# 0xEigenLabs/eigen-zkvm

Hardware: AMD Instinct MI355X
Metric: Goldilocks NTT GElems/s + BN254 G1 MSM Mpts/s; starky prove ms at 2^24 rows (higher is better)
Workload: dtype u64 (Goldilocks, canonical)

## Files before the change

eigen-zkvm_amd/csrc/ntt.hip:

```cpp
#include "zk_internal.h"
#include "ntt_reg.hip.h"
#include <map>
#include <mutex>
#include <vector>

namespace zk {

namespace {

constexpr int NTT_TILE = 4096;
constexpr int TW_LO_BITS = 12;
constexpr int TW_LO = 1 << TW_LO_BITS;

struct PassParams {
    const u64* in;
    u64* out;
    const u64* w256;
    const u64* tw_lo;
    const u64* tw_hi;
    const u64* tw_mid;
    u64 pre_scale;
    u32 dshift;
    const u64* sc_lo;
    const u64* sc_hi;
    u64 sc_step;
    u64 out_scale;
    u64 inner;
    u64 valid_in;
    u64 s_np;
    u32 np;
    u32 log_s;
    u32 has_tw;
};

__device__ __forceinline__ u64 tab2(const u64* __restrict__ lo, const u64* __restrict__ hi, u64 e) {
    return gl::mul_tw_nc(hi[e >> TW_LO_BITS], lo[e & (TW_LO - 1)]);
}

template <int LOGA, int LOGB, bool KMODE, bool INV>
__global__ __launch_bounds__(NTT_TILE / 16) void ntt_pass_kernel(const PassParams P) {
    constexpr int LOGR = LOGA + LOGB, R = 1 << LOGR, RA = 1 << LOGA, RB = 1 << LOGB;
    constexpr int C = NTT_TILE / R;
    constexpr int GA = 16 / RA, GB = 16 / RB;
    constexpr int TG = R / 16;
    constexpr int PAD = KMODE ? 512 / R : 0;
    constexpr int ROW = RB * C + PAD;
    static_assert(LOGR >= 4 && LOGR <= 8 && LOGA <= 4 && LOGB <= 4, "tile shape");
    __shared__ u64 lds[RA * ROW];

    const int t = threadIdx.x;
    const u64 u0 = (u64)blockIdx.x * C;

    {
        const int c = t % C, ta = t / C;
        const u64 u = u0 + c;
        const bool live = u < P.inner;
        u64 x[GA][RA];
        const bool full = u0 + C <= P.inner && (u64)(R - 1) * P.inner + u0 + C <= P.valid_in;
        const u64* __restrict__ base = P.in + (u64)(ta * GA) * P.inner + (live ? u : 0);
        if (full) {
#pragma unroll
            for (int g = 0; g < GA; ++g)
#pragma unroll
                for (int ja = 0; ja < RA; ++ja) x[g][ja] = base[(u64)(ja * RB + g) * P.inner];
        } else {
#pragma unroll
            for (int g = 0; g < GA; ++g)
#pragma unroll
                for (int ja = 0; ja < RA; ++ja) {
                    const u64 off = (u64)(ja * RB + g) * P.inner;
                    const bool ok = live && (u64)(ta * GA) * P.inner + off + u < P.valid_in;
                    const u64 v = *(ok ? base + off : P.in);
                    x[g][ja] = ok ? v : 0;
                }
        }
#pragma unroll
        for (int g = 0; g < GA; ++g) ntt_reg<LOGA, INV>(x[g]);
        if (LOGR <= 6 && C >= 64 && LOGB > 0 && P.pre_scale == 1) {
            static_for<0, TG>([&](auto TA) {
                constexpr int ta_c = decltype(TA)::value;
                if (ta == ta_c) {
                    static_for<0, GA>([&](auto GI) {
                        constexpr int g = decltype(GI)::value, jb = ta_c * GA + g;
                        static_for<0, RA>([&](auto KA) {
                            constexpr int ka = decltype(KA)::value;
                            constexpr int e0 = (39 * (64 / (R > 64 ? 64 : R)) * jb * ka) % 192, e = INV ? (192 - e0) % 192 : e0;
                            u64 v = x[g][bitrev_c(ka, LOGA)];
                            if constexpr (e >= 96) v = gl::neg(gl::mul_pow2<e - 96>(v));
                            else v = gl::mul_pow2<e>(v);
                            lds[ka * ROW + jb * C + c] = v;
                        });
                    });
                }
            });
        } else
        {
#pragma unroll
            for (int g = 0; g < GA; ++g) {
                const int jb = ta * GA + g;
#pragma unroll
                for (int ka = 0; ka < RA; ++ka) {
                    u64 v = x[g][bitrev_c(ka, LOGA)];
                    if (LOGB > 0 && ka > 0) v = gl::mul_tw(v, P.w256[(jb * ka) << (8 - LOGR)]);
                    else if (P.pre_scale != 1) v = gl::mul_tw(v, P.pre_scale);
                    lds[ka * ROW + jb * C + c] = v;
                }
            }
        }
    }
    __syncthreads();
    {
        int c, tb;
        if (KMODE) { tb = t % TG; c = t / TG; } else { c = t % C; tb = t / C; }
        const u64 u = u0 + c;
        u64 y[GB][RB];
#pragma unroll
        for (int g = 0; g < GB; ++g) {
            const int ka = tb + g * TG;
#pragma unroll
            for (int jb = 0; jb < RB; ++jb) y[g][jb] = lds[ka * ROW + jb * C + c];
        }
        const u64 uc = u < P.inner ? u : 0;
        u64 p, rem;
        if (P.np == 1) { p = uc >> P.log_s; rem = uc & (((u64)1 << P.log_s) - 1); }
        else if ((P.inner >> 32) == 0) { const u32 p32 = (u32)uc / (u32)P.s_np; p = p32; rem = (u32)uc - p32 * (u32)P.s_np; }
        else
        { p = uc / P.s_np; rem = uc - p * P.s_np; }
        u64 tw[GB][RB];
        if (P.tw_mid) {
#pragma unroll
            for (int g = 0; g < GB; ++g) {
                const int ka = tb + g * TG;
#pragma unroll
                for (int kb = 0; kb < RB; ++kb) tw[g][kb] = P.tw_mid[((p * (u64)(RA * kb + ka)) << P.log_s) >> P.dshift];
            }
        }
#pragma unroll
        for (int g = 0; g < GB; ++g) ntt_reg<LOGB, INV>(y[g]);
        if (u >= P.inner) return;

        u64* __restrict__ outp = P.out + p * R * P.s_np + rem;
        const u64 kstride = P.s_np;
        const u64 row_q = !P.sc_lo ? 0 : P.np == 1 ? rem : (P.inner >> 32) == 0 ? (u64)((u32)rem / P.np) : rem / P.np;
        if (P.tw_mid) {
#pragma unroll
            for (int g = 0; g < GB; ++g) {
                const int ka = tb + g * TG;
#pragma unroll
                for (int kb = 0; kb < RB; ++kb) {
                    u64 v = y[g][bitrev_c(kb, LOGB)];
                    v = gl::mul_tw(v, tw[g][kb]);
                    outp[(u64)(RA * kb + ka) * kstride] = v;
                }
            }
            return;
        }
        u64 tw_step = 1;
        if (P.has_tw) tw_step = tab2(P.tw_lo, P.tw_hi, (p * RA) << P.log_s);
#pragma unroll
        for (int g = 0; g < GB; ++g) {
            const int ka = tb + g * TG;
            u64 f = P.out_scale;
            if (P.has_tw) f = tab2(P.tw_lo, P.tw_hi, (p * ka) << P.log_s);
            if (P.sc_lo) f = tab2(P.sc_lo, P.sc_hi, ((u64)ka << P.log_s) + row_q);
            const bool scaled = P.has_tw || P.sc_lo || P.out_scale != 1;
            const u64 fstep = P.sc_lo ? P.sc_step : tw_step;
#pragma unroll
            for (int kb = 0; kb < RB; ++kb) {
                u64 v = y[g][bitrev_c(kb, LOGB)];
                if (scaled) {
                    v = gl::mul_tw(v, f);
                    if (kb + 1 < RB) f = gl::mul_tw_nc(f, fstep);
                }
                outp[(u64)(RA * kb + ka) * kstride] = v;
            }
        }
    }
}

__global__ void ntt_small_kernel(const u64* in, u64* out, u32 np, u32 n_in, u32 n, u64 w, u64 g, u64 cst) {
    const u32 tid = blockIdx.x * blockDim.x + threadIdx.x;
    if (tid >= n * np) return;
    const u32 k = tid / np, c = tid % np;
    const u64 wk = gl::pow(w, k);
    u64 acc = 0, cur = 1;
    for (u32 i = 0; i < n_in; ++i) { acc = gl::add(acc, gl::mul(in[(u64)i * np + c], cur)); cur = gl::mul(cur, wk); }
    out[(u64)k * np + c] = gl::mul(acc, gl::mul(cst, gl::pow(g, k)));
}

struct Tables { DevConst w256, w256s, lo, hi, mid; u32 dshift = 0; };
struct ScaleTables { DevConst lo, hi; };

std::mutex g_mu;
auto& g_tables = *new std::map<std::pair<int, std::pair<u32, int>>, Tables>;
auto& g_scales = *new std::map<std::pair<int, std::pair<u32, u64>>, ScaleTables>;

void two_level(u64 base, u64 cst, u32 nbits, std::vector<u64>& lo, std::vector<u64>& hi) {
    lo.resize(TW_LO);
    u64 c = cst;
    for (int i = 0; i < TW_LO; ++i) { lo[i] = c; c = gl::hmul(c, base); }
    size_t nh = nbits > (u32)TW_LO_BITS ? (size_t)1 << (nbits - TW_LO_BITS) : 1;
    hi.resize(nh);
    u64 step = gl::hpow(base, TW_LO);
    c = 1;
    for (size_t i = 0; i < nh; ++i) { hi[i] = c; c = gl::hmul(c, step); }
}

const Tables& get_tables(u32 nbits, bool inverse) {
    int dev; ZK_HIP(hipGetDevice(&dev));
    std::lock_guard<std::mutex> lk(g_mu);
    auto key = std::make_pair(dev, std::make_pair(nbits, (int)inverse));
    auto it = g_tables.find(key);
    if (it != g_tables.end()) return it->second;
    u64 w = gl::hroot(nbits), w8 = gl::hroot(8);
    if (inverse) { w = gl::hinv(w); w8 = gl::hinv(w8); }
    std::vector<u64> t256(256), lo, hi;
    u64 c = 1;
    for (int i = 0; i < 256; ++i) { t256[i] = c; c = gl::hmul(c, w8); }
    two_level(w, 1, nbits, lo, hi);
    Tables T; T.w256 = DevConst(t256); T.lo = DevConst(lo); T.hi = DevConst(hi);
    if (inverse) {
        const u64 ninv = gl::hinv((1ull << nbits) % GL_P);
        std::vector<u64> t256s(256);
        for (int i = 0; i < 256; ++i) t256s[i] = gl::hmul(t256[i], ninv);
        T.w256s = DevConst(t256s);
    }
    {
        T.dshift = nbits > 16 ? nbits - 16 : 0;
        const size_t nm = (size_t)1 << (nbits - T.dshift);
        std::vector<u64> mid(nm);
        const u64 step = gl::hpow(w, 1ull << T.dshift);
        c = 1;
        for (size_t i = 0; i < nm; ++i) { mid[i] = c; c = gl::hmul(c, step); }
        T.mid = DevConst(mid);
    }
    return g_tables.emplace(key, std::move(T)).first->second;
}

const ScaleTables& get_scale(u32 nbits, u64 g, u64 cst) {
    int dev; ZK_HIP(hipGetDevice(&dev));
    std::lock_guard<std::mutex> lk(g_mu);
    auto key = std::make_pair(dev, std::make_pair(nbits, g));
    auto it = g_scales.find(key);
    if (it != g_scales.end()) return it->second;
    std::vector<u64> lo, hi;
    two_level(g, cst, nbits, lo, hi);
    ScaleTables S; S.lo = DevConst(lo); S.hi = DevConst(hi);
    return g_scales.emplace(key, std::move(S)).first->second;
}

template <int LOGA, int LOGB>
void launch_pass(const PassParams& P, bool kmode, bool inverse, hipStream_t st) {
    constexpr int C = NTT_TILE >> (LOGA + LOGB);
    const u64 blocks = (P.inner + C - 1) / C;
    ZK_REQUIRE(blocks < (1ull << 31), "ntt: grid too large");
    const dim3 g((u32)blocks), b(NTT_TILE / 16);
    const int variant = (kmode ? 2 : 0) | (inverse ? 1 : 0);
#define ZK_PASS(K, I) hipLaunchKernelGGL((ntt_pass_kernel<LOGA, LOGB, K, I>), g, b, 0, st, P)
    switch (variant) {
        case 0: ZK_PASS(false, false); break; case 1: ZK_PASS(false, true); break;
        case 2: ZK_PASS(true, false); break;  default: ZK_PASS(true, true); break;
    }
#undef ZK_PASS
    ZK_HIP(hipGetLastError());
}

void launch_pass_logr(int logr, const PassParams& P, bool kmode, bool inverse, hipStream_t st) {
    switch (logr) {
        case 4: launch_pass<2, 2>(P, kmode, inverse, st); break;
        case 5: launch_pass<3, 2>(P, kmode, inverse, st); break;
        case 6: launch_pass<3, 3>(P, kmode, inverse, st); break;
        case 7: launch_pass<4, 3>(P, kmode, inverse, st); break;
        case 8: launch_pass<4, 4>(P, kmode, inverse, st); break;
        default: throw Error("ntt: unsupported pass radix");
    }
}

std::vector<int> plan(u32 nbits) {
    std::vector<int> r;
    if (nbits < 4) return r;
    int np = (nbits + 7) / 8;
    int base = nbits / np, extra = nbits % np;
    for (int i = 0; i < np; ++i) r.push_back(base + (i < extra ? 1 : 0));
    return r;
}

struct Scale { bool on = false; u64 g = 1, cst = 1; };

void run_transform(const u64* in, u64* a, u64* b,
                   u32 n_pols, u32 nbits, u64 valid_rows, bool inverse, Scale sc, u64 out_scale, hipStream_t st) {
    const u64 n = 1ull << nbits;
    if (nbits < 4) {
        u64 w = gl::hroot(nbits);
        if (inverse) w = gl::hinv(w);
        u64 cst = sc.on ? sc.cst : out_scale;
        u64 g = sc.on ? sc.g : 1;
        u32 total = (u32)(n * n_pols);
        hipLaunchKernelGGL(ntt_small_kernel, dim3((total + 255) / 256), dim3(256), 0, st, in, a, n_pols,
                           (u32)valid_rows, (u32)n, w, g, cst);
        ZK_HIP(hipGetLastError());
        return;
    }
    const std::vector<int> radices = plan(nbits);
    const int np = (int)radices.size();
    const Tables& T = get_tables(nbits, inverse);
    const ScaleTables* S = sc.on ? &get_scale(nbits, sc.g, sc.cst) : nullptr;
    u32 log_s = 0;
    const u64* cur = in;
    for (int i = 0; i < np; ++i) {
        const int logr = radices[i];
        u64* dstbuf = ((np - 1 - i) % 2 == 0) ? a : b;
        const bool last = (i == np - 1);
        PassParams P{};
        P.in = cur; P.out = dstbuf;
        P.w256 = T.w256.u(); P.tw_lo = T.lo.u(); P.tw_hi = T.hi.u();
        P.sc_lo = (last && sc.on) ? S->lo.u() : nullptr;
        P.sc_hi = (last && sc.on) ? S->hi.u() : nullptr;
        const int loga = (logr + 1) / 2;
        P.sc_step = (last && sc.on) ? gl::hpow(sc.g, (1ull << loga) << log_s) : 1;
        P.out_scale = 1; P.pre_scale = 1;
        if (last && !sc.on && out_scale != 1) {
            ZK_REQUIRE(inverse && out_scale == gl::hinv(n % GL_P), "ntt: unsupported constant scaling");
            P.w256 = T.w256s.u(); P.pre_scale = out_scale;
        }
        P.inner = (n >> logr) * n_pols;
        P.valid_in = (i == 0) ? valid_rows * n_pols : n * n_pols;
        P.s_np = ((u64)1 << log_s) * n_pols;
        P.np = n_pols;
        P.log_s = log_s;
        P.has_tw = last ? 0 : 1;
        P.dshift = T.dshift;
        P.tw_mid = (!last && log_s >= T.dshift) ? T.mid.u() : nullptr;
        const bool kmode = P.s_np < 16;
        launch_pass_logr(logr, P, kmode, inverse, st);
        cur = dstbuf;
        log_s += logr;
    }
}

}

int ntt_num_passes(uint32_t nbits) { return nbits < 4 ? 1 : (int)plan(nbits).size(); }

const u64* ntt_w256_table(bool inverse) { return get_tables(8, inverse).w256.u(); }

void ntt_dev(const u64* d_src, u64* d_dst, u64* d_tmp, uint32_t n_pols, uint32_t nbits, bool inverse, hipStream_t st) {
    ZK_REQUIRE(nbits <= 32, "ntt: nbits > 32");
    if (n_pols == 0) return;
    ZK_REQUIRE(d_src != d_dst, "ntt: dst may not alias src");
    u64 out_scale = inverse ? gl::hinv((1ull << nbits) % GL_P) : 1;
    run_transform(d_src, d_dst, d_tmp, n_pols, nbits, 1ull << nbits, inverse, Scale{}, out_scale, st);
}

void lde_dev(const u64* d_src, u64* d_dst, u64* d_tmp, uint32_t n_pols, uint32_t nbits, uint32_t nbits_ext, hipStream_t st) {
    ZK_REQUIRE(nbits_ext <= 32 && nbits <= nbits_ext, "lde: need nbits <= nbits_ext <= 32");
    if (n_pols == 0) return;
    ZK_REQUIRE(d_src != d_dst, "lde: dst may not alias src");
    const u64 n = 1ull << nbits;
    Scale sc; sc.on = true; sc.g = 49; sc.cst = gl::hinv(n % GL_P);
    const int fwd_passes = ntt_num_passes(nbits_ext);
    u64* first_fwd_out = ((fwd_passes - 1) % 2 == 0) ? d_dst : d_tmp;
    u64* coef = (first_fwd_out == d_dst) ? d_tmp : d_dst;
    u64* other = (coef == d_dst) ? d_tmp : d_dst;
    run_transform(d_src, coef, other, n_pols, nbits, n, true, sc, 1, st);
    run_transform(coef, d_dst, d_tmp, n_pols, nbits_ext, n, false, Scale{}, 1, st);
}

}
```

Before: 81.06.

## Prefetch twiddle/scale factors before first stage and break serial factor chain

Issues the global-table loads for the output twiddle/coset factors right after the input loads, so their latency overlaps the first radix stage. Per-column step factors are precomputed cooperatively into a new shared array, replacing the serial per-kb multiply chain with independent multiplies. The scale step is now derived from a table entry times the inverse of the constant. It also adds 32-bit byte-offset addressing for tw_mid loads and for output stores when the problem is small. Costs are extra LDS and registers per block, which may lower occupancy.

```diff
diff --git a/eigen-zkvm_amd/csrc/ntt.hip b/eigen-zkvm_amd/csrc/ntt.hip
--- a/eigen-zkvm_amd/csrc/ntt.hip
+++ b/eigen-zkvm_amd/csrc/ntt.hip
@@ -2,6 +2,7 @@
 #include "ntt_reg.hip.h"
 #include <map>
 #include <mutex>
+#include <type_traits>
 #include <vector>
 
 namespace zk {
@@ -23,7 +24,7 @@
     u32 dshift;
     const u64* sc_lo;
     const u64* sc_hi;
-    u64 sc_step;
+    u64 sc_cinv;
     u64 out_scale;
     u64 inner;
     u64 valid_in;
@@ -47,9 +48,50 @@
     constexpr int ROW = RB * C + PAD;
     static_assert(LOGR >= 4 && LOGR <= 8 && LOGA <= 4 && LOGB <= 4, "tile shape");
     __shared__ u64 lds[RA * ROW];
+    __shared__ u64 sfac[RB * C];
 
     const int t = threadIdx.x;
     const u64 u0 = (u64)blockIdx.x * C;
+
+    auto split = [&](u64 u, u64& p, u64& rem) {
+        const u64 uc = u < P.inner ? u : 0;
+        if (P.np == 1) { p = uc >> P.log_s; rem = uc & (((u64)1 << P.log_s) - 1); }
+        else if ((P.inner >> 32) == 0) { const u32 p32 = (u32)uc / (u32)P.s_np; p = p32; rem = (u32)uc - p32 * (u32)P.s_np; }
+        else
+        { p = uc / P.s_np; rem = uc - p * P.s_np; }
+    };
+    auto row_of = [&](u64 rem) { return P.np == 1 ? rem : (P.inner >> 32) == 0 ? (u64)((u32)rem / P.np) : rem / P.np; };
+    const bool small = ((P.inner * R) >> 29) == 0;
+    int cB, tb;
+    if (KMODE) { tb = t % TG; cB = t / TG; } else { cB = t % C; tb = t / C; }
+
+    const bool split_f = (P.has_tw && !P.tw_mid) || P.sc_lo;
+    u64 fa_hi[GB], fa_lo[GB], fs_hi[GA], fs_lo[GA], fa[GB];
+#pragma unroll
+    for (int g = 0; g < GB; ++g) fa_hi[g] = fa_lo[g] = fa[g] = 1;
+#pragma unroll
+    for (int m = 0; m < GA; ++m) fs_hi[m] = fs_lo[m] = 1;
+    auto issue_factor_loads = [&]() {
+        const u64* __restrict__ lo = P.sc_lo ? P.sc_lo : P.tw_lo;
+        const u64* __restrict__ hi = P.sc_lo ? P.sc_hi : P.tw_hi;
+        u64 p, rem;
+        split(u0 + cB, p, rem);
+        const u32 rq = P.sc_lo ? (u32)row_of(rem) : 0;
+#pragma unroll
+        for (int g = 0; g < GB; ++g) {
+            const u32 ka = tb + g * TG;
+            const u32 e = P.sc_lo ? (ka << P.log_s) + rq : ((u32)p * ka) << P.log_s;
+            fa_hi[g] = hi[e >> TW_LO_BITS]; fa_lo[g] = lo[e & (TW_LO - 1)];
+        }
+#pragma unroll
+        for (int m = 0; m < GA; ++m) {
+            const int i = t + m * (NTT_TILE / 16);
+            const u32 kb = i / C;
+            split(u0 + i % C, p, rem);
+            const u32 e = P.sc_lo ? (RA * kb) << P.log_s : ((u32)p * (RA * kb)) << P.log_s;
+            fs_hi[m] = hi[e >> TW_LO_BITS]; fs_lo[m] = lo[e & (TW_LO - 1)];
+        }
+    };
 
     {
         const int c = t % C, ta = t / C;
@@ -74,6 +116,7 @@
                     x[g][ja] = ok ? v : 0;
                 }
         }
+        if (split_f) issue_factor_loads();
 #pragma unroll
         for (int g = 0; g < GA; ++g) ntt_reg<LOGA, INV>(x[g]);
         if (LOGR <= 6 && C >= 64 && LOGB > 0 && P.pre_scale == 1) {
@@ -108,10 +151,19 @@
             }
         }
     }
+    if (split_f) {
+#pragma unroll
+        for (int m = 0; m < GA; ++m) {
+            u64 sv = gl::mul_tw_nc(fs_hi[m], fs_lo[m]);
+            if (P.sc_lo) sv = gl::mul_tw_nc(sv, P.sc_cinv);
+            sfac[t + m * (NTT_TILE / 16)] = sv;
+        }
+#pragma unroll
+        for (int g = 0; g < GB; ++g) fa[g] = gl::mul_tw_nc(fa_hi[g], fa_lo[g]);
+    }
     __syncthreads();
     {
-        int c, tb;
-        if (KMODE) { tb = t % TG; c = t / TG; } else { c = t % C; tb = t / C; }
+        const int c = cB;
         const u64 u = u0 + c;
         u64 y[GB][RB];
 #pragma unroll
@@ -120,61 +172,59 @@
 #pragma unroll
             for (int jb = 0; jb < RB; ++jb) y[g][jb] = lds[ka * ROW + jb * C + c];
         }
-        const u64 uc = u < P.inner ? u : 0;
         u64 p, rem;
-        if (P.np == 1) { p = uc >> P.log_s; rem = uc & (((u64)1 << P.log_s) - 1); }
-        else if ((P.inner >> 32) == 0) { const u32 p32 = (u32)uc / (u32)P.s_np; p = p32; rem = (u32)uc - p32 * (u32)P.s_np; }
-        else
-        { p = uc / P.s_np; rem = uc - p * P.s_np; }
+        split(u, p, rem);
         u64 tw[GB][RB];
         if (P.tw_mid) {
+            const u32 sh = P.log_s - P.dshift, istep = (((u32)p * RA) << sh) * 8;
 #pragma unroll
             for (int g = 0; g < GB; ++g) {
-                const int ka = tb + g * TG;
-#pragma unroll
-                for (int kb = 0; kb < RB; ++kb) tw[g][kb] = P.tw_mid[((p * (u64)(RA * kb + ka)) << P.log_s) >> P.dshift];
+                const u32 ka = tb + g * TG, i0 = (((u32)p * ka) << sh) * 8;
+#pragma unroll
+                for (int kb = 0; kb < RB; ++kb) tw[g][kb] = *(const u64*)((const char*)P.tw_mid + (u32)(i0 + kb * istep));
             }
         }
 #pragma unroll
         for (int g = 0; g < GB; ++g) ntt_reg<LOGB, INV>(y[g]);
         if (u >= P.inner) return;
 
-        u64* __restrict__ outp = P.out + p * R * P.s_np + rem;
-        const u64 kstride = P.s_np;
-        const u64 row_q = !P.sc_lo ? 0 : P.np == 1 ? rem : (P.inner >> 32) == 0 ? (u64)((u32)rem / P.np) : rem / P.np;
-        if (P.tw_mid) {
-#pragma unroll
-            for (int g = 0; g < GB; ++g) {
-                const int ka = tb + g * TG;
-#pragma unroll
-                for (int kb = 0; kb < RB; ++kb) {
-                    u64 v = y[g][bitrev_c(kb, LOGB)];
-                    v = gl::mul_tw(v, tw[g][kb]);
-                    outp[(u64)(RA * kb + ka) * kstride] = v;
-                }
+        auto finish = [&](auto small_c) {
+            constexpr bool SMALL = decltype(small_c)::value;
+            u64* __restrict__ outp = P.out + p * R * P.s_np + rem;
+            const u64 kstride = P.s_np;
+            const u32 b0 = ((u32)p * R * (u32)P.s_np + (u32)rem) * 8, bstep = RA * (u32)P.s_np * 8;
+            auto put = [&](int g, int kb, u64 v) {
+                const u32 ka = tb + g * TG;
+                if constexpr (SMALL) *(u64*)((char*)P.out + (u32)(b0 + ka * (u32)P.s_np * 8 + kb * bstep)) = v;
+                else outp[(u64)(RA * kb + ka) * kstride] = v;
+            };
+            if (P.tw_mid) {
+#pragma unroll
+                for (int g = 0; g < GB; ++g)
+#pragma unroll
+                    for (int kb = 0; kb < RB; ++kb) put(g, kb, gl::mul_tw(y[g][bitrev_c(kb, LOGB)], tw[g][kb]));
+            } else if (split_f) {
+#pragma unroll
+                for (int g = 0; g < GB; ++g)
+#pragma unroll
+                    for (int kb = 0; kb < RB; ++kb) {
+                        const u64 f = kb == 0 ? fa[g] : gl::mul_tw_nc(fa[g], sfac[kb * C + c]);
+                        put(g, kb, gl::mul_tw(y[g][bitrev_c(kb, LOGB)], f));
+                    }
+            } else if (P.out_scale != 1) {
+#pragma unroll
+                for (int g = 0; g < GB; ++g)
+#pragma unroll
+                    for (int kb = 0; kb < RB; ++kb) put(g, kb, gl::mul_tw(y[g][bitrev_c(kb, LOGB)], P.out_scale));
+            } else {
+#pragma unroll
+                for (int g = 0; g < GB; ++g)
+#pragma unroll
+                    for (int kb = 0; kb < RB; ++kb) put(g, kb, y[g][bitrev_c(kb, LOGB)]);
             }
-            return;
-        }
-        u64 tw_step = 1;
-        if (P.has_tw) tw_step = tab2(P.tw_lo, P.tw_hi, (p * RA) << P.log_s);
-#pragma unroll
-        for (int g = 0; g < GB; ++g) {
-            const int ka = tb + g * TG;
-            u64 f = P.out_scale;
-            if (P.has_tw) f = tab2(P.tw_lo, P.tw_hi, (p * ka) << P.log_s);
-            if (P.sc_lo) f = tab2(P.sc_lo, P.sc_hi, ((u64)ka << P.log_s) + row_q);
-            const bool scaled = P.has_tw || P.sc_lo || P.out_scale != 1;
-            const u64 fstep = P.sc_lo ? P.sc_step : tw_step;
-#pragma unroll
-            for (int kb = 0; kb < RB; ++kb) {
-                u64 v = y[g][bitrev_c(kb, LOGB)];
-                if (scaled) {
-                    v = gl::mul_tw(v, f);
-                    if (kb + 1 < RB) f = gl::mul_tw_nc(f, fstep);
-                }
-                outp[(u64)(RA * kb + ka) * kstride] = v;
-            }
-        }
+        };
+        if (small) finish(std::true_type{});
+        else finish(std::false_type{});
     }
 }
 
@@ -316,8 +366,7 @@
         P.w256 = T.w256.u(); P.tw_lo = T.lo.u(); P.tw_hi = T.hi.u();
         P.sc_lo = (last && sc.on) ? S->lo.u() : nullptr;
         P.sc_hi = (last && sc.on) ? S->hi.u() : nullptr;
-        const int loga = (logr + 1) / 2;
-        P.sc_step = (last && sc.on) ? gl::hpow(sc.g, (1ull << loga) << log_s) : 1;
+        P.sc_cinv = (last && sc.on) ? gl::hinv(sc.cst) : 1;
         P.out_scale = 1; P.pre_scale = 1;
         if (last && !sc.on && out_scale != 1) {
             ZK_REQUIRE(inverse && out_scale == gl::hinv(n % GL_P), "ntt: unsupported constant scaling");
```

New measurement: 82.85, median of 6. 1.02x the previous value.
